# yongduosui/CAL

Measured on AMD Instinct MI355X. Metric: graphs/sec (train step) on SPMotif b=0.9 batch=128, higher is better.
Workload: dtype f32; 1 GPU; spmotif_b0.9_causalgcn_h128_l3_bs128; model=CausalGCN, batch_per_gpu=128, global_batch=128, hidden=128, layers=3, node_num=7, launch=graph(8 steps per graph launch, remainder 3), parallelism=dp1, resident_batches=8

## Files before the change

### cal_amd/csrc/engine.hip

```cpp
#include <string.h>
#include <hip/hip_ext.h>

#include <algorithm>
#include <type_traits>
#include <vector>

#include "engine_kernels.hpp"
#include "engine_readout.hpp"
#include "engine_gconv.hpp"
#include "engine_gconv_bwd.hpp"
#include "engine_ggat.hpp"
#include "engine_plan.hpp"
#include "engine_attbwd.hpp"
#include "engine_ro_step.hpp"
#include "engine_gin.hpp"
#include "engine_ggin.hpp"
#include "engine_feat.hpp"
#include "engine_gwide.hpp"
#include "engine_attwide.hpp"

namespace cal {

constexpr int MAX_LAYERS = 6;
constexpr int MAX_SLABS = 24;
// ... 129 lines not shown
    int o_cw, o_cb, o_ow, o_ob;
    int o_fc1_w[3], o_fc1_b[3], o_fc2_w[3], o_fc2_b[3];
    BNSlot bn[MAX_LAYERS + 9];
    int nbn;
    int a_convb[MAX_LAYERS], a_cb, a_ob, a_dwn, a_dwe, a_db1, a_db2, a_sync, arena_n, bn_plane;
    char* ws; size_t ws_bytes;
    int64_t capN, capE, capB;
    float *h, *z, *zco, *hco, *anode, *pq, *att, *dis_unit, *dis_co, *pooled, *pcnt, *xco, *y1, *zl, *logp, *stats, *zpart;
    int adam_fused;
    int ro_rows;
    int striped;
    int fold_zero;
    int bn0_dirty_host;
    int gwide;
    int ro_step;
    float *dzl, *dyh1, *dy1, *dxh, *dpool, *dZco, *gn, *gself, *ddeg, *dl, *dzco, *dXhco, *dZ, *dzi, *dXh, *slabs;
    size_t slab_floats;
    double* arena;
    double* parts; size_t parts_doubles;
    hipStream_t side; hipEvent_t ev_fork[24], ev_join[24];
    int *rowptr_dst, *nbr_dst, *eid_dst, *rowptr_src, *nbr_src, *eid_src, *row32, *col32, *work, *status, *gptr, *iperm, *eptr;
    float* wslot;
    float* coef_src;
    float* coef;
    int max_nodes, max_edges;
    const int64_t *node_ptr, *edge_ptr;
    const int64_t* tile_gptr; int ntiles;
    int K; float gat_p, gat_slope;
    uint64_t gat_seed[MAX_LAYERS];
    unsigned long long* gat_ctr;
// ... 26 lines not shown
              hipStream_t stream);
}

extern "C" int64_t cal_gat_bwd_ws(int64_t N, int64_t E, int64_t K, int64_t D);

CAL_EXPORT void* cal_engine_create(int64_t F, int64_t H, int64_t C, int64_t L) {
    if (H % 4 != 0 || H > 256 || H < 4 || L < 0 || L > MAX_LAYERS || F < 1 || C < 1 || C > 64) {
        set_error("cal_engine_create: unsupported shape (need hidden %% 4 == 0, hidden <= 256, layers <= %d, classes <= 64)", MAX_LAYERS);
        return nullptr;
    }
    Engine* e = new Engine();
    memset(e, 0, sizeof(Engine));
    if (hipHostMalloc((void**)&e->host_status, 64, hipHostMallocMapped | hipHostMallocCoherent) == hipSuccess) *e->host_status = 0;
    else { (void)hipGetLastError(); e->host_status = nullptr; }
    { const char* v = getenv("CAL_AMD_RO_STEP"); e->ro_step = !(v && v[0] == '0'); }
    { const char* v = getenv("CAL_AMD_RO_ROWS"); e->ro_rows = !(v && v[0] == '0'); }
    { const char* v = getenv("CAL_AMD_STRIPED"); e->striped = !(v && v[0] == '0'); }
    { const char* v = getenv("CAL_AMD_GWIDE"); e->gwide = !(v && v[0] == '0'); }
    { const char* v = getenv("CAL_AMD_FOLD_ZERO"); e->fold_zero = !(v && v[0] == '0'); }
    e->bn0_dirty_host = 1;
    {
        int dev = 0, cus = 0;
        if (hipGetDevice(&dev) != hipSuccess || hipDeviceGetAttribute(&cus, hipDeviceAttributeMultiprocessorCount, dev) != hipSuccess) cus = 0;
        if (cus < 3 * ((int)H / RO_CW) + 8) e->ro_step = 0;
        e->num_cus = cus > 0 ? cus : 256;
        if (cus < 3 * ((int)H / RO_CW) * RBK_MAXRB + 8) e->ro_rows = 0;
    }
    { const char* v = getenv("CAL_AMD_ADAM_FUSED"); e->adam_fused = !(v && v[0] == '0'); }
    e->F = (int)F; e->H = (int)H; e->C = (int)C; e->L = (int)L;
    e->loop_w = 1.f;
// ... 950 lines not shown
    SpmmBranch b0{e->zco, e->hco, e->P + e->o_cb, e->att, e->dis_co, Acc(), Acc(), nullptr, nullptr, nullptr};
    SpmmBranch b1{e->zco + NH, e->hco + NH, e->P + e->o_ob, e->att + E, e->dis_co + N, Acc(), Acc(), nullptr, nullptr, nullptr};
    RC(launch_espmm(st, gd, SpmmBranch2{{b0, b1}}, 2, 1, e->loop_w, N, H, spmm_rpb(H, false)));
    CAL_CHECK_LAUNCH("k_espmm(co)"); STAGE();
    RC(launch_pool2(c)); STAGE();
    return 0;
}

int fwd_readout(Ctx& c) {
    Engine* e = c.e;
    const int B = c.B, H = e->H, C = e->C, L = e->L;
    hipStream_t st = c.st;
    if (c.r.ro == Readout::OneLaunch || c.r.ro == Readout::Rows) {
        RoStepArgs sa;
        memset(&sa, 0, sizeof(sa));
        sa.a = make_ro(c); sa.zpart = e->zpart; sa.sync = reinterpret_cast<int*>(e->arena + e->a_sync); sa.status = e->status;
        if (c.r.ro == Readout::OneLaunch) {
            hipLaunchKernelGGL(k_ro_step<false>, dim3(3, H / RO_CW), dim3(256), 0, st, sa);
        } else {
            const int nrb = cdiv(B, RS_B), nch = H / RO_CW;
            sa.nrb = nrb;
            sa.xch = parts_alloc(c, (size_t)3 * nch * RBK_XCH);
            if (!sa.xch) return no_parts();
            sa.gw1_slab = e->slabs; sa.gw2_slab = e->slabs + (size_t)3 * nrb * H * H;
            hipLaunchKernelGGL(k_ro_step<true>, dim3(3, nch, nrb), dim3(256), 0, st, sa);
        }
        CAL_CHECK_LAUNCH("k_ro_step"); STAGE();
        return 0;
    }
    if (c.r.ro == Readout::FourKernel) {
        const RoArgs ra = make_ro(c);
        hipLaunchKernelGGL(k_ro_fwd_a, dim3(3, H / RO_CW), dim3(256), 0, st, ra);
        CAL_CHECK_LAUNCH("k_ro_fwd_a"); STAGE();
        hipLaunchKernelGGL(k_ro_fwd_b, dim3(3, cdiv(B, RO_RB)), dim3(256), 0, st, ra);
        CAL_CHECK_LAUNCH("k_ro_fwd_b"); STAGE();
        if (!c.want_grad) {
            hipLaunchKernelGGL(k_ro_loss, dim3(3), dim3(256), 0, st, ra);
            CAL_CHECK_LAUNCH("k_ro_loss");
        }
        return 0;
// ... 982 lines not shown
```

### cal_amd/csrc/engine_ro_step.hpp

```cpp
#pragma once
#include "engine_readout.hpp"

namespace cal {

constexpr int RS_B = 128;
constexpr int RS_K = 128;
constexpr int RS_LD = RS_K + 4;

struct RoStepArgs {
    RoArgs a;
    float* zpart;
    int* sync;
    int* status;
    double* xch;
    float* gw1_slab; float* gw2_slab;
    int nrb;
};
constexpr int RBK_MAXRB = 4;
constexpr int RBK_N0 = 2 * RS_K, RBK_N1 = 2 * RO_CW, RBK_N2 = 2 * (RO_CW + 1), RBK_N3 = 4 * 64;
constexpr int RBK_O1 = RBK_MAXRB * RBK_N0, RBK_O2 = RBK_O1 + RBK_MAXRB * RBK_N1, RBK_O3 = RBK_O2 + RBK_MAXRB * RBK_N2;
constexpr int RBK_XCH = RBK_O3 + RBK_MAXRB * RBK_N3;
constexpr int RBK_SYNC_INTS = 3 * RBK_MAXRB * 2 + 3 * (RS_K / RO_CW) * 4;

__device__ __forceinline__ void ro_step_arrive(int* ctr) {
// ... 3 lines not shown
__device__ __forceinline__ void ro_step_wait(int* ctr, int n, int* status) {
    if (threadIdx.x == 0) {
        int spins = 0;
        while (__hip_atomic_load(ctr, __ATOMIC_RELAXED, __HIP_MEMORY_SCOPE_AGENT) < n) {
            if (++spins > (1 << 21)) { if (status) atomicOr(status, 256); break; }
            __builtin_amdgcn_s_sleep(1);
        }
        __builtin_amdgcn_fence(__ATOMIC_ACQUIRE, "agent");
    }
    __syncthreads();
}
__device__ __forceinline__ void ro_step_barrier(int* ctr, int n, int* status) {
    ro_step_arrive(ctr);
    ro_step_wait(ctr, n, status);
}
template <int NT, bool BN>
__device__ __forceinline__ void ro_mfma_rowk_nt(int kred, const float* X, int ld, int nrow, const float* Wr, const float* sc,
                                                const float* sh, ro_f32x4 (&acc)[4]) {
    const int l = threadIdx.x & 63, w = threadIdx.x >> 6, lr = l & 15, lk = l >> 4;
    const float* ar[NT];
#pragma unroll
    for (int t = 0; t < NT; ++t) ar[t] = X + min((w + 4 * t) * 16 + lr, nrow - 1) * ld + 4 * lk;
    const float* br = Wr + lr * ld + 4 * lk;
    float4 a4[NT], b4, s4 = make_float4(1.f, 1.f, 1.f, 1.f), h4 = make_float4(0.f, 0.f, 0.f, 0.f);
    auto fetch = [&](int k0, float4 (&a)[NT], float4& b, float4& s, float4& h) {
#pragma unroll
        for (int t = 0; t < NT; ++t) a[t] = *reinterpret_cast<const float4*>(ar[t] + k0);
        b = *reinterpret_cast<const float4*>(br + k0);
        if (BN) { s = *reinterpret_cast<const float4*>(sc + k0 + 4 * lk); h = *reinterpret_cast<const float4*>(sh + k0 + 4 * lk); }
    };
    fetch(0, a4, b4, s4, h4);
    for (int k0 = 0; k0 < kred; k0 += 16) {
        float4 an[NT], bn, sn = s4, hn = h4;
        fetch(min(k0 + 16, kred - 16), an, bn, sn, hn);
        const float bb[4] = {b4.x, b4.y, b4.z, b4.w}, ss[4] = {s4.x, s4.y, s4.z, s4.w}, hh[4] = {h4.x, h4.y, h4.z, h4.w};
#pragma unroll
        for (int j = 0; j < 4; ++j)
#pragma unroll
            for (int t = 0; t < NT; ++t) {
                const float aa[4] = {a4[t].x, a4[t].y, a4[t].z, a4[t].w};
                acc[t] = __builtin_amdgcn_mfma_f32_16x16x4f32(BN ? fmaf(aa[j], ss[j], hh[j]) : aa[j], bb[j], acc[t], 0, 0, 0);
            }
#pragma unroll
        for (int t = 0; t < NT; ++t) a4[t] = an[t];
        b4 = bn; s4 = sn; h4 = hn;
    }
}
template <bool BN>
__device__ __forceinline__ void ro_mfma_rowk(int ntiles, int kred, const float* X, int ld, int nrow, const float* Wr, const float* sc,
                                             const float* sh, ro_f32x4 (&acc)[4]) {
    switch ((ntiles + 3) / 4) {
        case 1: ro_mfma_rowk_nt<1, BN>(kred, X, ld, nrow, Wr, sc, sh, acc); break;
        case 2: ro_mfma_rowk_nt<2, BN>(kred, X, ld, nrow, Wr, sc, sh, acc); break;
        case 3: ro_mfma_rowk_nt<3, BN>(kred, X, ld, nrow, Wr, sc, sh, acc); break;
        default: ro_mfma_rowk_nt<4, BN>(kred, X, ld, nrow, Wr, sc, sh, acc); break;
    }
}

template <int NV>
__device__ __forceinline__ void rbk_total(double (&v)[NV], int t, int n, double* xs, int nrb, int rb, int* ctr, int* status) {
    if (t < n) {
#pragma unroll
        for (int q = 0; q < NV; ++q) xs[(size_t)rb * NV * n + q * n + t] = v[q];
    }
    ro_step_barrier(ctr, nrb, status);
    if (t < n) {
#pragma unroll
        for (int q = 0; q < NV; ++q) {
            double tot = 0.0;
            for (int r = 0; r < nrb; ++r) tot += xs[(size_t)r * NV * n + q * n + t];
            v[q] = tot;
        }
    }
}

template <bool RBK>
__global__ void __launch_bounds__(256) k_ro_step(const RoStepArgs sa) {
    warm_kernargs<(sizeof(RoStepArgs) < 1024 ? sizeof(RoStepArgs) : 1024)>();
    const RoArgs& a = sa.a;
    __shared__ __attribute__((aligned(16))) float Xs[RS_B * RS_LD];
    __shared__ __attribute__((aligned(16))) float Ws[RO_CW * RS_LD];
    __shared__ __attribute__((aligned(16))) float W1t[RO_CW * RS_LD];
    __shared__ __attribute__((aligned(16))) float scratch[2 * RS_B * RO_CW];
    __shared__ __attribute__((aligned(16))) float xn[RS_B * RO_CW];
    __shared__ __attribute__((aligned(16))) float y1c[RS_B * RO_CW];
    __shared__ __attribute__((aligned(16))) float zs[2048];
    __shared__ __attribute__((aligned(16))) float W2c[64 * RO_CW];
    __shared__ __attribute__((aligned(16))) float sc_s[RS_K], sh_s[RS_K], mean1_s[RS_K], rstd1_s[RS_K];
    __shared__ int perm_s[256];
    __shared__ double red[2][256];
    __shared__ float c2[6][RO_CW];
    __shared__ double lossp_s[2];
    const int hd = blockIdx.x, ch = blockIdx.y, j0 = ch * RO_CW, nch = gridDim.y;
    const int Bt = a.B, rb = RBK ? (int)blockIdx.z : 0, r0 = rb * RS_B, nrb = RBK ? sa.nrb : 1;
    const int B = RBK ? min(RS_B, Bt - r0) : Bt, K = a.H, C = a.C, ld = RS_LD, K4 = K / 4, BC = B * C, BCt = Bt * C;
    int* const cbar = RBK ? sa.sync + (hd * RBK_MAXRB + rb) * 2 : sa.sync + hd * 2;
    int* const gbar = sa.sync + 3 * RBK_MAXRB * 2 + (hd * nch + ch) * 4;
    double* const xch = RBK ? sa.xch + (size_t)(hd * nch + ch) * RBK_XCH : nullptr;
    const RoHead& h = a.h[hd];
    const int l = threadIdx.x & 63, w = threadIdx.x >> 6, j = l & 15, lk = l >> 4;
    const int rl = threadIdx.x / RO_CW;
    float* dyh = scratch;
    float* yn = scratch + RS_B * RO_CW;
    double (*red8)[256] = reinterpret_cast<double (*)[256]>(scratch);
    const int B16 = (B + 15) & ~15, ntiles = B16 / 16;
    const bool duty_out = ch == 1 % nch, duty_loss = ch == 2 % nch, duty_db2 = ch == 3 % nch,
               duty_xco = ch == 4 % nch, duty_run1 = ch == 5 % nch;

    RO_CLK(40);
    const bool colfix = 256 % K4 == 0;
    float sf[4] = {0.f, 0.f, 0.f, 0.f}, qf[4] = {0.f, 0.f, 0.f, 0.f}, pvt[4] = {0.f, 0.f, 0.f, 0.f};
    int nst = 0;
    auto add_stats = [&](const float4 v) {
        const float vv[4] = {v.x, v.y, v.z, v.w};
#pragma unroll
        for (int c = 0; c < 4; ++c) {
            pvt[c] = nst == 0 ? vv[c] : pvt[c];
            const float d = vv[c] - pvt[c];
            sf[c] += d; qf[c] = fmaf(d, d, qf[c]);
        }
        ++nst;
    };
    int pv = hd == 2 ? (int)a.perm[r0 + min((int)threadIdx.x, B - 1)] : 0;
    float g2 = h.bn2.gamma[j0 + j], b2n = h.bn2.beta[j0 + j], rm2 = h.bn2.run_mean[j0 + j], rv2 = h.bn2.run_var[j0 + j];
    float bias1 = h.b1[j0 + j];
    float rm1 = h.bn1.run_mean[min((int)threadIdx.x, K - 1)], rv1 = h.bn1.run_var[min((int)threadIdx.x, K - 1)];
    int ylab = (int)a.y[r0 + min((int)threadIdx.x, B - 1)];
    {
        RoBatch<float4, 2> bw;
        RoBatch<float, 8> bt;
        RoBatch<float, 4> bw2;
        ro_issue(bw, RO_CW, K4, [&](int jj, int c) { return *reinterpret_cast<const float4*>(h.W1 + (size_t)(j0 + jj) * K + c * 4); });
        ro_issue(bt, K, RO_CW, [&](int jj, int ii) { return h.W1[(size_t)jj * K + j0 + ii]; });
        ro_issue(bw2, C, RO_CW, [&](int c, int jj) { return h.W2[(size_t)c * K + j0 + jj]; });
        auto commit_weights = [&]() {
            ro_commit(bw, RO_CW, K4, [&](int jj, int c, const float4 v) { *reinterpret_cast<float4*>(Ws + jj * ld + c * 4) = v; });
            ro_commit(bt, K, RO_CW, [&](int jj, int ii, float v) { W1t[ii * ld + jj] = v; });
            ro_commit(bw2, C, RO_CW, [&](int c, int jj, float v) { W2c[c * RO_CW + jj] = v; });
            asm volatile("" : "+v"(g2), "+v"(b2n), "+v"(rm2), "+v"(rv2), "+v"(bias1), "+v"(ylab), "+v"(rm1), "+v"(rv1));
        };
        RoBatch<float4, 16> bx;
        if (hd == 2) {
            asm volatile("" : "+v"(pv));
            perm_s[threadIdx.x] = pv;
            __syncthreads();
            RoBatch<float4, 16> bp;
            ro_issue(bx, B, K4, [&](int b, int c) { return *reinterpret_cast<const float4*>(a.pooled + (size_t)(Bt + r0 + b) * K + c * 4); });
            ro_issue(bp, B, K4, [&](int b, int c) { return *reinterpret_cast<const float4*>(a.pooled + (size_t)perm_s[b] * K + c * 4); });
            commit_weights();
            ro_commit2(bx, bp, B, K4, [&](int b, int c, const float4 o, const float4 p) {
                const float4 v = make_float4(p.x + o.x, p.y + o.y, p.z + o.z, p.w + o.w);
                *reinterpret_cast<float4*>(Xs + b * ld + c * 4) = v;
                if (colfix) add_stats(v);
                if (duty_xco) *reinterpret_cast<float4*>(a.xco + (size_t)(r0 + b) * K + c * 4) = v;
            });
            if (duty_xco && (int)threadIdx.x < B) a.iperm[pv] = r0 + threadIdx.x;
        } else {
            const float* src = a.pooled + (hd == 0 ? (size_t)0 : (size_t)Bt * K) + (size_t)r0 * K;
            ro_issue(bx, B, K4, [&](int b, int c) { return *reinterpret_cast<const float4*>(src + (size_t)b * K + c * 4); });
            commit_weights();
            ro_commit(bx, B, K4, [&](int b, int c, const float4 v) {
                *reinterpret_cast<float4*>(Xs + b * ld + c * 4) = v;
                if (colfix) add_stats(v);
            });
        }
        __syncthreads();
    }
    RO_CLK(41);
    {
        const int np = 256 / K4, cg = threadIdx.x % K4, part = threadIdx.x / K4;
        if (!colfix && part < np) {
#pragma unroll 4
            for (int b = part; b < B; b += np) add_stats(*reinterpret_cast<const float4*>(Xs + b * ld + 4 * cg));
        }
#pragma unroll
        for (int c = 0; c < 4; ++c) {
            const double P = (double)pvt[c], S0 = (double)sf[c], n0 = (double)nst;
            red8[c][threadIdx.x] = S0 + n0 * P;
            red8[4 + c][threadIdx.x] = (double)qf[c] + 2.0 * P * S0 + n0 * P * P;
        }
        __syncthreads();
        double SQ[2] = {0.0, 0.0};
        if ((int)threadIdx.x < K) {
            const int g = threadIdx.x >> 2, c = threadIdx.x & 3;
            for (int p = 0; p < np; ++p) { SQ[0] += red8[c][p * K4 + g]; SQ[1] += red8[4 + c][p * K4 + g]; }
        }
        if (RBK) rbk_total<2>(SQ, threadIdx.x, K, xch, nrb, rb, gbar + 0, sa.status);
        if ((int)threadIdx.x < K) {
            const int k = threadIdx.x;
            const double S = SQ[0], Q = SQ[1];
            float sc, sh, mean, rstd;
            ro_bn_from_sums(h.bn1, k, S, Q, sc, sh, mean, rstd);
            sc_s[k] = sc; sh_s[k] = sh; mean1_s[k] = mean; rstd1_s[k] = rstd;
            if (duty_run1 && rb == 0) {
                const double m = S * (double)h.bn1.inv_n;
                double v = Q * (double)h.bn1.inv_n - m * m;
                if (v < 0.0) v = 0.0;
                h.bn1.run_mean[k] = 0.9f * rm1 + 0.1f * (float)m;
                h.bn1.run_var[k] = 0.9f * rv1 + 0.1f * (float)(v * (double)h.bn1.unbias);
                if (k == 0 && h.bn1.nbt) *h.bn1.nbt += 1;
            }
        }
        __syncthreads();
    }
    RO_CLK(42);
    for (int idx = threadIdx.x; idx < B16 * RO_CW; idx += 256) {
        const int b = idx / RO_CW, ii = idx % RO_CW;
        xn[idx] = b < B ? Xs[b * ld + j0 + ii] : 0.f;
    }
    ro_f32x4 acc[4] = {};
    ro_mfma_rowk<true>(ntiles, K, Xs, ld, B, Ws, sc_s, sh_s, acc);
    float s1 = 0.f, s2 = 0.f, pv2 = 0.f;
    int n2 = 0;
#pragma unroll
    for (int t = 0; t < 4; ++t)
#pragma unroll
        for (int r = 0; r < 4; ++r) {
            const int b = (w + 4 * t) * 16 + lk * 4 + r;
            const float v = b < B ? fmaxf(acc[t][r] + bias1, 0.f) : 0.f;
            if (b < B) y1c[b * RO_CW + j] = v;
            pv2 = (b < B && n2 == 0) ? v : pv2;
            const float d = b < B ? v - pv2 : 0.f;
            n2 += b < B ? 1 : 0;
            s1 += d; s2 = fmaf(d, d, s2);
        }
    RO_CLK(43);
    {
        const double P = (double)pv2, S0 = (double)s1, n0 = (double)n2;
        red[0][threadIdx.x] = S0 + n0 * P; red[1][threadIdx.x] = (double)s2 + 2.0 * P * S0 + n0 * P * P;
    }
    __syncthreads();
    double SQ2[2] = {0.0, 0.0};
    if (threadIdx.x < RO_CW)
        for (int p = 0; p < 16; ++p) { SQ2[0] += red[0][p * RO_CW + threadIdx.x]; SQ2[1] += red[1][p * RO_CW + threadIdx.x]; }
    if (RBK) rbk_total<2>(SQ2, threadIdx.x, RO_CW, xch + RBK_O1, nrb, rb, gbar + 1, sa.status);
    if (threadIdx.x < RO_CW) {
        const double S = SQ2[0], Q = SQ2[1];
        if (rb == 0) { h.st2_sum[j0 + threadIdx.x] = S; h.st2_sq[j0 + threadIdx.x] = Q; }
        const double m = S * (double)h.bn2.inv_n;
        double v = Q * (double)h.bn2.inv_n - m * m;
        if (v < 0.0) v = 0.0;
        c2[0][threadIdx.x] = (float)m; c2[1][threadIdx.x] = 1.0f / sqrtf((float)v + h.bn2.eps);
        c2[2][threadIdx.x] = g2; c2[3][threadIdx.x] = b2n;
        if (rb == 0) {
            h.bn2.run_mean[j0 + threadIdx.x] = 0.9f * rm2 + 0.1f * (float)m;
            h.bn2.run_var[j0 + threadIdx.x] = 0.9f * rv2 + 0.1f * (float)(v * (double)h.bn2.unbias);
            if (ch == 0 && threadIdx.x == 0 && h.bn2.nbt) *h.bn2.nbt += 1;
        }
    }
    __syncthreads();
    const float mean2 = c2[0][j], rstd2 = c2[1][j], gam2 = c2[2][j], bet2 = c2[3][j];
    {
        const float sc = gam2 * rstd2, sh = bet2 - mean2 * sc;
        for (int b = rl; b < B; b += 16) yn[b * RO_CW + j] = fmaf(y1c[b * RO_CW + j], sc, sh);
    }
    __syncthreads();
    {
        float* zp = sa.zpart + ((size_t)hd * nch + ch) * BCt + (size_t)r0 * C;
        for (int o = threadIdx.x; o < BC; o += 256) {
            const int b = o / C, c = o % C;
            const float4* yr = reinterpret_cast<const float4*>(yn + b * RO_CW);
            const float4* wr = reinterpret_cast<const float4*>(W2c + c * RO_CW);
            zp[o] = dot4(yr[3], wr[3], dot4(yr[2], wr[2], dot4(yr[1], wr[1], dot4(yr[0], wr[0], 0.f))));
        }
    }
    RO_CLK(44);
    ro_step_barrier(cbar, nch, sa.status);
    RO_CLK(45);

    for (int o0 = 0; o0 < BC; o0 += 512) {
        float pz[2][8], bz[2];
#pragma unroll
        for (int v = 0; v < 2; ++v) {
            const int o = min(o0 + v * 256 + (int)threadIdx.x, BC - 1);
            bz[v] = h.b2[o % C];
#pragma unroll
            for (int p = 0; p < 8; ++p) pz[v][p] = sa.zpart[((size_t)hd * nch + min(p, nch - 1)) * BCt + (size_t)r0 * C + o];
        }
#pragma unroll
        for (int v = 0; v < 2; ++v) {
            ro_pin(bz[v]);
#pragma unroll
            for (int p = 0; p < 8; ++p) ro_pin(pz[v][p]);
        }
#pragma unroll
        for (int v = 0; v < 2; ++v) {
            const int o = o0 + v * 256 + (int)threadIdx.x;
            float z = 0.f;
#pragma unroll
            for (int p = 0; p < 8; ++p) z += p < nch ? pz[v][p] : 0.f;
            z += bz[v];
            if (o < BC) {
                zs[o] = z;
                if (duty_out) a.zl[(size_t)hd * BCt + (size_t)r0 * C + o] = z;
            }
        }
    }
    __syncthreads();
    float lv = 0.f, cv = 0.f;
    if ((int)threadIdx.x < B) {
        const int b = threadIdx.x;
        const float u = 1.0f / (float)C, invB = 1.0f / (float)Bt, logu = logf(u);
// ... 30 lines not shown
            for (int k = 0; k < C; ++k) m = fmaxf(m, zr[k]);
            float se = 0.f;
            for (int k = 0; k < C; ++k) se += expf(zr[k] - m);
            const float lse = m + logf(se);
            for (int k = 0; k < C; ++k) finish(k, zr[k], lse);
        }
        lv = (float)lrow; cv = arg == yy ? 1.f : 0.f;
    }
    if (duty_loss) {
        double ls = (double)lv, cs = (double)cv;
#pragma unroll
        for (int o = 32; o > 0; o >>= 1) { ls += __shfl_xor(ls, o, 64); cs += __shfl_xor(cs, o, 64); }
        if (l == 0) { red[0][w] = ls; red[1][w] = cs; }
        __syncthreads();
        if (threadIdx.x == 0) {
            const double lsum = red[0][0] + red[0][1] + red[0][2] + red[0][3], csum = red[1][0] + red[1][1] + red[1][2] + red[1][3];
            if (RBK) { lossp_s[0] = lsum; lossp_s[1] = csum; }
            else {
                a.stats[1 + hd] = (float)(lsum / (double)Bt);
                a.stats[hd == 1 ? 4 : (hd == 0 ? 5 : 6)] = (float)csum;
            }
        }
    }
    __syncthreads();
    RO_CLK(46);
    const float* dzs = zs;
    double db1_keep = 0.0, db2_keep = 0.0;
    {
        float t1f = 0.f, t2f = 0.f;
        float dq[8] = {0.f, 0.f, 0.f, 0.f, 0.f, 0.f, 0.f, 0.f};
        for (int c = 0; c < C; ++c) {
            const float wc2 = W2c[c * RO_CW + j];
            float dzv[8];
#pragma unroll
            for (int qq = 0; qq < 8; ++qq) dzv[qq] = dzs[min(rl + 16 * qq, B - 1) * C + c];
#pragma unroll
            for (int qq = 0; qq < 8; ++qq) dq[qq] = fmaf(dzv[qq], wc2, dq[qq]);
        }
#pragma unroll
        for (int qq = 0; qq < 8; ++qq) {
            const int b = rl + 16 * qq;
            const float yv = y1c[min(b, B - 1) * RO_CW + j];
            if (b < B) {
                const float n = (yv - mean2) * rstd2;
                dyh[b * RO_CW + j] = dq[qq];
                t1f += dq[qq]; t2f = fmaf(dq[qq], n, t2f);
            }
        }
        double t1 = (double)t1f, t2 = (double)t2f;
        red[0][threadIdx.x] = t1; red[1][threadIdx.x] = t2;
        __syncthreads();
        if (rl == 0) for (int p = 1; p < 16; ++p) { t1 += red[0][p * RO_CW + j]; t2 += red[1][p * RO_CW + j]; }
        if (RBK) {
            double tt[2] = {rl == 0 ? t1 : 0.0, rl == 0 ? t2 : 0.0};
            if (threadIdx.x == RO_CW) { tt[0] = duty_loss ? lossp_s[0] : 0.0; tt[1] = duty_loss ? lossp_s[1] : 0.0; }
            rbk_total<2>(tt, threadIdx.x, RO_CW + 1, xch + RBK_O2, nrb, rb, gbar + 2, sa.status);
            t1 = tt[0]; t2 = tt[1];
            if (threadIdx.x == RO_CW && duty_loss && rb == 0) {
                a.stats[1 + hd] = (float)(tt[0] / (double)Bt);
                a.stats[hd == 1 ? 4 : (hd == 0 ? 5 : 6)] = (float)tt[1];
            }
        }
        if (rl == 0) {
            if (rb == 0) { h.d2_sum[j0 + j] = t1; h.d2_prod[j0 + j] = t2; }
            c2[4][j] = (float)(t1 * (double)h.bn2.inv_n); c2[5][j] = (float)(t2 * (double)h.bn2.inv_n);
        }
        __syncthreads();
        const float m1 = c2[4][j], m2 = c2[5][j], gs = gam2 * rstd2;
        float sbf = 0.f;
#pragma unroll
        for (int qq = 0; qq < 8; ++qq) {
            const int b = rl + 16 * qq;
            if (b < B) {
                const float yv = y1c[b * RO_CW + j];
                const float n = (yv - mean2) * rstd2;
                const float dy = yv > 0.f ? gs * (dyh[b * RO_CW + j] - m1 - n * m2) : 0.f;
                a.dy1[((size_t)hd * Bt + r0 + b) * K + j0 + j] = dy;
                sbf += dy;
            }
        }
        double sb = (double)sbf;
        red[0][threadIdx.x] = sb;
        __syncthreads();
        if (rl == 0) {
            for (int p = 1; p < 16; ++p) sb += red[0][p * RO_CW + j];
            if (RBK) db1_keep = sb; else h.db1[j0 + j] = sb;
        }
    }
    RO_CLK(47);
    ro_step_arrive(cbar + 1);
    RO_CLK(48);
    ro_step_wait(cbar + 1, nch, sa.status);
    RO_CLK(49);
    float* Ds = Xs;
    RoBatch<float4, 16> bd;
    ro_issue(bd, B, K4, [&](int b, int c) { return *reinterpret_cast<const float4*>(a.dy1 + ((size_t)hd * Bt + r0 + b) * K + c * 4); });
    if (duty_db2) {
        const int np = 256 / C, c = threadIdx.x % C, part = threadIdx.x / C;
        double sdz = 0.0;
        if (part < np) for (int b = part; b < B; b += np) sdz += (double)dzs[b * C + c];
        red[0][threadIdx.x] = sdz;
        __syncthreads();
        if (part == 0) {
            for (int p2 = 1; p2 < np; ++p2) sdz += red[0][p2 * C + c];
            if (RBK) db2_keep = sdz; else h.db2[c] = sdz;
        }
        __syncthreads();
    }
    {
        const int nout = C * RO_CW;
        float* fred = dyh;
        for (int o0 = 0; o0 < nout; o0 += 256) {
            const int no = min(256, nout - o0), np = 256 / no;
            const int o = o0 + threadIdx.x % no, part = threadIdx.x / no;
            const int c = o / RO_CW, jj = o % RO_CW;
            float accw = 0.f;
            if (part < np) {
#pragma unroll 4
                for (int b = part; b < B; b += np) accw = fmaf(dzs[b * C + c], yn[b * RO_CW + jj], accw);
            }
            __syncthreads();
            fred[threadIdx.x] = accw;
            __syncthreads();
            if (part == 0) {
                for (int p = 1; p < np; ++p) accw += fred[p * no + threadIdx.x];
                (RBK ? sa.gw2_slab + ((size_t)hd * nrb + rb) * C * K : h.gW2)[(size_t)c * K + j0 + jj] = accw;
            }
        }
    }
    ro_commit(bd, B, K4, [&](int b, int c, const float4 v) { *reinterpret_cast<float4*>(Ds + b * ld + c * 4) = v; });
    for (int idx = threadIdx.x; idx < (B16 - B) * ld; idx += 256) Ds[B * ld + idx] = 0.f;
    __syncthreads();
    RO_CLK(50);
    const int i = j, i0 = j0;
    const float mean1 = mean1_s[i0 + i], rstd1 = rstd1_s[i0 + i], gs1 = sc_s[i0 + i], sh1 = sh_s[i0 + i];
    ro_f32x4 dacc[4] = {};
    ro_mfma_rowk<false>(ntiles, K, Ds, ld, B, W1t, nullptr, nullptr, dacc);
    float u1 = 0.f, u2 = 0.f;
#pragma unroll
    for (int t = 0; t < 4; ++t)
#pragma unroll
        for (int r = 0; r < 4; ++r) {
            const int b = (w + 4 * t) * 16 + lk * 4 + r;
            const float n = (xn[min(b, B16 - 1) * RO_CW + i] - mean1) * rstd1;
            const float dv = b < B ? dacc[t][r] : 0.f;
            u1 += dv; u2 = fmaf(dv, n, u2);
        }
    red[0][threadIdx.x] = (double)u1; red[1][threadIdx.x] = (double)u2;
    __syncthreads();
    {
        double uu[4] = {0.0, 0.0, 0.0, 0.0};
        if (threadIdx.x < RO_CW)
            for (int p = 0; p < 16; ++p) { uu[0] += red[0][p * RO_CW + threadIdx.x]; uu[1] += red[1][p * RO_CW + threadIdx.x]; }
        if (RBK) {
            uu[2] = threadIdx.x < RO_CW ? db1_keep : 0.0;
            uu[3] = (duty_db2 && (int)threadIdx.x < C) ? db2_keep : 0.0;
            rbk_total<4>(uu, threadIdx.x, 64, xch + RBK_O3, nrb, rb, gbar + 3, sa.status);
            if (rb == 0) {
                if (threadIdx.x < RO_CW) h.db1[j0 + threadIdx.x] = uu[2];
                if (duty_db2 && (int)threadIdx.x < C) h.db2[threadIdx.x] = uu[3];
            }
        }
        if (threadIdx.x < RO_CW) {
            const double S = uu[0], Q = uu[1];
            if (rb == 0) { h.d1_sum[i0 + threadIdx.x] = S; h.d1_prod[i0 + threadIdx.x] = Q; }
            c2[4][threadIdx.x] = (float)(S * (double)h.bn1.inv_n); c2[5][threadIdx.x] = (float)(Q * (double)h.bn1.inv_n);
        }
    }
    __syncthreads();
    {
        const float m1 = c2[4][i], m2 = c2[5][i];
#pragma unroll
        for (int t = 0; t < 4; ++t)
#pragma unroll
            for (int r = 0; r < 4; ++r) {
                const int b = (w + 4 * t) * 16 + lk * 4 + r;
                if (b < B) {
                    const float xr = xn[b * RO_CW + i];
                    const float n = (xr - mean1) * rstd1;
                    a.dxin[((size_t)hd * Bt + r0 + b) * K + i0 + i] = gs1 * (dacc[t][r] - m1 - n * m2);
                    xn[b * RO_CW + i] = fmaf(xr, gs1, sh1);
                }
            }
    }
    __syncthreads();
    RO_CLK(51);
    ro_f32x4 wacc[4] = {};
    ro_mfma_tiles(K / 16, B16, [&](int row, int k) { return Ds[k * ld + min(row, K - 1)]; },
                  [&](int k, int col) { return xn[k * RO_CW + col]; }, wacc);
#pragma unroll
    for (int t = 0; t < 4; ++t)
        if (w + 4 * t < K / 16) {
#pragma unroll
            for (int r = 0; r < 4; ++r)
                (RBK ? sa.gw1_slab + ((size_t)hd * nrb + rb) * K * K : h.gW1)[(size_t)((w + 4 * t) * 16 + lk * 4 + r) * K + i0 + i] = wacc[t][r];
        }
    RO_CLK(52);
}

}
```

Before: 580,400 graphs/s.

## Run readout step kernel with 8 waves, splitting MFMA K-reduction across wave halves

Templates k_ro_step on block size and adds a 512-thread variant, selected by default for the single-launch readout when batch exceeds 64. The two wave groups each compute half of the K (or batch) reduction in the MFMA GEMMs and combine partial accumulators through shared memory. Loads and reductions are re-strided to NT threads. This aims to cut the latency of a low-occupancy kernel that runs only 3×(H/RO_CW) blocks, at the cost of extra shared-memory combine passes and barriers.

```diff
diff --git a/cal_amd/csrc/engine.hip b/cal_amd/csrc/engine.hip
--- a/cal_amd/csrc/engine.hip
+++ b/cal_amd/csrc/engine.hip
@@ -167,6 +167,7 @@
     int bn0_dirty_host;
     int gwide;
     int ro_step;
+    int ro_step_nt;
     float *dzl, *dyh1, *dy1, *dxh, *dpool, *dZco, *gn, *gself, *ddeg, *dl, *dzco, *dXhco, *dZ, *dzi, *dXh, *slabs;
     size_t slab_floats;
     double* arena;
@@ -223,6 +224,7 @@
     if (hipHostMalloc((void**)&e->host_status, 64, hipHostMallocMapped | hipHostMallocCoherent) == hipSuccess) *e->host_status = 0;
     else { (void)hipGetLastError(); e->host_status = nullptr; }
     { const char* v = getenv("CAL_AMD_RO_STEP"); e->ro_step = !(v && v[0] == '0'); }
+    { const char* v = getenv("CAL_AMD_RO_STEP_NT"); const int n = v ? atoi(v) : 0; e->ro_step_nt = n == 256 || n == 512 ? n : 0; }
     { const char* v = getenv("CAL_AMD_RO_ROWS"); e->ro_rows = !(v && v[0] == '0'); }
     { const char* v = getenv("CAL_AMD_STRIPED"); e->striped = !(v && v[0] == '0'); }
     { const char* v = getenv("CAL_AMD_GWIDE"); e->gwide = !(v && v[0] == '0'); }
@@ -1203,16 +1205,19 @@
     if (c.r.ro == Readout::OneLaunch || c.r.ro == Readout::Rows) {
         RoStepArgs sa;
         memset(&sa, 0, sizeof(sa));
+        const int nt = e->ro_step_nt ? e->ro_step_nt : (c.r.ro == Readout::OneLaunch && B > RS_B / 2 ? 512 : 256);
         sa.a = make_ro(c); sa.zpart = e->zpart; sa.sync = reinterpret_cast<int*>(e->arena + e->a_sync); sa.status = e->status;
         if (c.r.ro == Readout::OneLaunch) {
-            hipLaunchKernelGGL(k_ro_step<false>, dim3(3, H / RO_CW), dim3(256), 0, st, sa);
+            if (nt == 512) hipLaunchKernelGGL((k_ro_step<false, 512>), dim3(3, H / RO_CW), dim3(512), 0, st, sa);
+            else hipLaunchKernelGGL((k_ro_step<false, 256>), dim3(3, H / RO_CW), dim3(256), 0, st, sa);
         } else {
             const int nrb = cdiv(B, RS_B), nch = H / RO_CW;
             sa.nrb = nrb;
             sa.xch = parts_alloc(c, (size_t)3 * nch * RBK_XCH);
             if (!sa.xch) return no_parts();
             sa.gw1_slab = e->slabs; sa.gw2_slab = e->slabs + (size_t)3 * nrb * H * H;
-            hipLaunchKernelGGL(k_ro_step<true>, dim3(3, nch, nrb), dim3(256), 0, st, sa);
+            if (nt == 512) hipLaunchKernelGGL((k_ro_step<true, 512>), dim3(3, nch, nrb), dim3(512), 0, st, sa);
+            else hipLaunchKernelGGL((k_ro_step<true, 256>), dim3(3, nch, nrb), dim3(256), 0, st, sa);
         }
         CAL_CHECK_LAUNCH("k_ro_step"); STAGE();
         return 0;
diff --git a/cal_amd/csrc/engine_ro_step.hpp b/cal_amd/csrc/engine_ro_step.hpp
--- a/cal_amd/csrc/engine_ro_step.hpp
+++ b/cal_amd/csrc/engine_ro_step.hpp
@@ -41,46 +41,60 @@
     ro_step_arrive(ctr);
     ro_step_wait(ctr, n, status);
 }
-template <int NT, bool BN>
-__device__ __forceinline__ void ro_mfma_rowk_nt(int kred, const float* X, int ld, int nrow, const float* Wr, const float* sc,
-                                                const float* sh, ro_f32x4 (&acc)[4]) {
-    const int l = threadIdx.x & 63, w = threadIdx.x >> 6, lr = l & 15, lk = l >> 4;
-    const float* ar[NT];
-#pragma unroll
-    for (int t = 0; t < NT; ++t) ar[t] = X + min((w + 4 * t) * 16 + lr, nrow - 1) * ld + 4 * lk;
-    const float* br = Wr + lr * ld + 4 * lk;
-    float4 a4[NT], b4, s4 = make_float4(1.f, 1.f, 1.f, 1.f), h4 = make_float4(0.f, 0.f, 0.f, 0.f);
-    auto fetch = [&](int k0, float4 (&a)[NT], float4& b, float4& s, float4& h) {
-#pragma unroll
-        for (int t = 0; t < NT; ++t) a[t] = *reinterpret_cast<const float4*>(ar[t] + k0);
+template <int TW, bool BN>
+__device__ __forceinline__ void ro_mfma_rowk_nt(int wq, int kbeg, int kred, const float* X, int ld, int nrow, const float* Wr,
+                                                const float* sc, const float* sh, ro_f32x4 (&acc)[4]) {
+    const int l = threadIdx.x & 63, lr = l & 15, lk = l >> 4;
+    const float* ar[TW];
+#pragma unroll
+    for (int t = 0; t < TW; ++t) ar[t] = X + min((wq + 4 * t) * 16 + lr, nrow - 1) * ld + kbeg + 4 * lk;
+    const float* br = Wr + lr * ld + kbeg + 4 * lk;
+    if (BN) { sc += kbeg + 4 * lk; sh += kbeg + 4 * lk; }
+    float4 a4[TW], b4, s4 = make_float4(1.f, 1.f, 1.f, 1.f), h4 = make_float4(0.f, 0.f, 0.f, 0.f);
+    auto fetch = [&](int k0, float4 (&a)[TW], float4& b, float4& s, float4& h) {
+#pragma unroll
+        for (int t = 0; t < TW; ++t) a[t] = *reinterpret_cast<const float4*>(ar[t] + k0);
         b = *reinterpret_cast<const float4*>(br + k0);
-        if (BN) { s = *reinterpret_cast<const float4*>(sc + k0 + 4 * lk); h = *reinterpret_cast<const float4*>(sh + k0 + 4 * lk); }
+        if (BN) { s = *reinterpret_cast<const float4*>(sc + k0); h = *reinterpret_cast<const float4*>(sh + k0); }
     };
     fetch(0, a4, b4, s4, h4);
     for (int k0 = 0; k0 < kred; k0 += 16) {
-        float4 an[NT], bn, sn = s4, hn = h4;
+        float4 an[TW], bn, sn = s4, hn = h4;
         fetch(min(k0 + 16, kred - 16), an, bn, sn, hn);
         const float bb[4] = {b4.x, b4.y, b4.z, b4.w}, ss[4] = {s4.x, s4.y, s4.z, s4.w}, hh[4] = {h4.x, h4.y, h4.z, h4.w};
 #pragma unroll
         for (int j = 0; j < 4; ++j)
 #pragma unroll
-            for (int t = 0; t < NT; ++t) {
+            for (int t = 0; t < TW; ++t) {
                 const float aa[4] = {a4[t].x, a4[t].y, a4[t].z, a4[t].w};
                 acc[t] = __builtin_amdgcn_mfma_f32_16x16x4f32(BN ? fmaf(aa[j], ss[j], hh[j]) : aa[j], bb[j], acc[t], 0, 0, 0);
             }
 #pragma unroll
-        for (int t = 0; t < NT; ++t) a4[t] = an[t];
+        for (int t = 0; t < TW; ++t) a4[t] = an[t];
         b4 = bn; s4 = sn; h4 = hn;
     }
 }
 template <bool BN>
-__device__ __forceinline__ void ro_mfma_rowk(int ntiles, int kred, const float* X, int ld, int nrow, const float* Wr, const float* sc,
-                                             const float* sh, ro_f32x4 (&acc)[4]) {
+__device__ __forceinline__ void ro_mfma_rowk(int wq, int ntiles, int kbeg, int kred, const float* X, int ld, int nrow, const float* Wr,
+                                             const float* sc, const float* sh, ro_f32x4 (&acc)[4]) {
     switch ((ntiles + 3) / 4) {
-        case 1: ro_mfma_rowk_nt<1, BN>(kred, X, ld, nrow, Wr, sc, sh, acc); break;
-        case 2: ro_mfma_rowk_nt<2, BN>(kred, X, ld, nrow, Wr, sc, sh, acc); break;
-        case 3: ro_mfma_rowk_nt<3, BN>(kred, X, ld, nrow, Wr, sc, sh, acc); break;
-        default: ro_mfma_rowk_nt<4, BN>(kred, X, ld, nrow, Wr, sc, sh, acc); break;
+        case 1: ro_mfma_rowk_nt<1, BN>(wq, kbeg, kred, X, ld, nrow, Wr, sc, sh, acc); break;
+        case 2: ro_mfma_rowk_nt<2, BN>(wq, kbeg, kred, X, ld, nrow, Wr, sc, sh, acc); break;
+        case 3: ro_mfma_rowk_nt<3, BN>(wq, kbeg, kred, X, ld, nrow, Wr, sc, sh, acc); break;
+        default: ro_mfma_rowk_nt<4, BN>(wq, kbeg, kred, X, ld, nrow, Wr, sc, sh, acc); break;
+    }
+}
+
+__device__ __forceinline__ void ro_half_combine(int wq, int kh, int ntw, float* park, ro_f32x4 (&acc)[4]) {
+    ro_f32x4* slot = reinterpret_cast<ro_f32x4*>(park) + (wq * 4) * 64 + (threadIdx.x & 63);
+    if (kh == 1) {
+#pragma unroll
+        for (int t = 0; t < 4; ++t) if (t < ntw) slot[t * 64] = acc[t];
+    }
+    __syncthreads();
+    if (kh == 0) {
+#pragma unroll
+        for (int t = 0; t < 4; ++t) if (t < ntw) acc[t] += slot[t * 64];
     }
 }
 
@@ -101,8 +115,11 @@
     }
 }
 
-template <bool RBK>
-__global__ void __launch_bounds__(256) k_ro_step(const RoStepArgs sa) {
+template <bool RBK, int NT>
+__global__ void __launch_bounds__(NT) k_ro_step(const RoStepArgs sa) {
+    static_assert(NT == 256 || NT == 512, "k_ro_step: 4 or 8 waves");
+    constexpr int NRP = NT / RO_CW;
+    constexpr int XU = RS_B * (RS_K / 4) / NT;
     warm_kernargs<(sizeof(RoStepArgs) < 1024 ? sizeof(RoStepArgs) : 1024)>();
     const RoArgs& a = sa.a;
     __shared__ __attribute__((aligned(16))) float Xs[RS_B * RS_LD];
@@ -114,8 +131,8 @@
     __shared__ __attribute__((aligned(16))) float zs[2048];
     __shared__ __attribute__((aligned(16))) float W2c[64 * RO_CW];
     __shared__ __attribute__((aligned(16))) float sc_s[RS_K], sh_s[RS_K], mean1_s[RS_K], rstd1_s[RS_K];
-    __shared__ int perm_s[256];
-    __shared__ double red[2][256];
+    __shared__ int perm_s[RS_B];
+    __shared__ double red[2][NT];
     __shared__ float c2[6][RO_CW];
     __shared__ double lossp_s[2];
     const int hd = blockIdx.x, ch = blockIdx.y, j0 = ch * RO_CW, nch = gridDim.y;
@@ -126,16 +143,19 @@
     double* const xch = RBK ? sa.xch + (size_t)(hd * nch + ch) * RBK_XCH : nullptr;
     const RoHead& h = a.h[hd];
     const int l = threadIdx.x & 63, w = threadIdx.x >> 6, j = l & 15, lk = l >> 4;
+    const int wq = w & 3, kh = NT == 512 ? w >> 2 : 0;
+    const bool own = kh == 0;
     const int rl = threadIdx.x / RO_CW;
     float* dyh = scratch;
     float* yn = scratch + RS_B * RO_CW;
-    double (*red8)[256] = reinterpret_cast<double (*)[256]>(scratch);
-    const int B16 = (B + 15) & ~15, ntiles = B16 / 16;
+    double (*red8s)[NT] = reinterpret_cast<double (*)[NT]>(scratch);
+    auto red8q = [&](int c) { return reinterpret_cast<double*>(c < 2 ? xn : y1c) + (c & 1) * NT; };
+    const int B16 = (B + 15) & ~15, ntiles = B16 / 16, ntw = (ntiles + 3) / 4;
     const bool duty_out = ch == 1 % nch, duty_loss = ch == 2 % nch, duty_db2 = ch == 3 % nch,
                duty_xco = ch == 4 % nch, duty_run1 = ch == 5 % nch;
 
     RO_CLK(40);
-    const bool colfix = 256 % K4 == 0;
+    const bool colfix = NT % K4 == 0;
     float sf[4] = {0.f, 0.f, 0.f, 0.f}, qf[4] = {0.f, 0.f, 0.f, 0.f}, pvt[4] = {0.f, 0.f, 0.f, 0.f};
     int nst = 0;
     auto add_stats = [&](const float4 v) {
@@ -154,28 +174,28 @@
     float rm1 = h.bn1.run_mean[min((int)threadIdx.x, K - 1)], rv1 = h.bn1.run_var[min((int)threadIdx.x, K - 1)];
     int ylab = (int)a.y[r0 + min((int)threadIdx.x, B - 1)];
     {
-        RoBatch<float4, 2> bw;
-        RoBatch<float, 8> bt;
-        RoBatch<float, 4> bw2;
-        ro_issue(bw, RO_CW, K4, [&](int jj, int c) { return *reinterpret_cast<const float4*>(h.W1 + (size_t)(j0 + jj) * K + c * 4); });
-        ro_issue(bt, K, RO_CW, [&](int jj, int ii) { return h.W1[(size_t)jj * K + j0 + ii]; });
-        ro_issue(bw2, C, RO_CW, [&](int c, int jj) { return h.W2[(size_t)c * K + j0 + jj]; });
+        RoBatch<float4, 512 / NT> bw;
+        RoBatch<float, 2048 / NT> bt;
+        RoBatch<float, 1024 / NT> bw2;
+        ro_issue<NT>(bw, RO_CW, K4, [&](int jj, int c) { return *reinterpret_cast<const float4*>(h.W1 + (size_t)(j0 + jj) * K + c * 4); });
+        ro_issue<NT>(bt, K, RO_CW, [&](int jj, int ii) { return h.W1[(size_t)jj * K + j0 + ii]; });
+        ro_issue<NT>(bw2, C, RO_CW, [&](int c, int jj) { return h.W2[(size_t)c * K + j0 + jj]; });
         auto commit_weights = [&]() {
-            ro_commit(bw, RO_CW, K4, [&](int jj, int c, const float4 v) { *reinterpret_cast<float4*>(Ws + jj * ld + c * 4) = v; });
-            ro_commit(bt, K, RO_CW, [&](int jj, int ii, float v) { W1t[ii * ld + jj] = v; });
-            ro_commit(bw2, C, RO_CW, [&](int c, int jj, float v) { W2c[c * RO_CW + jj] = v; });
+            ro_commit<NT>(bw, RO_CW, K4, [&](int jj, int c, const float4 v) { *reinterpret_cast<float4*>(Ws + jj * ld + c * 4) = v; });
+            ro_commit<NT>(bt, K, RO_CW, [&](int jj, int ii, float v) { W1t[ii * ld + jj] = v; });
+            ro_commit<NT>(bw2, C, RO_CW, [&](int c, int jj, float v) { W2c[c * RO_CW + jj] = v; });
             asm volatile("" : "+v"(g2), "+v"(b2n), "+v"(rm2), "+v"(rv2), "+v"(bias1), "+v"(ylab), "+v"(rm1), "+v"(rv1));
         };
-        RoBatch<float4, 16> bx;
+        RoBatch<float4, XU> bx;
         if (hd == 2) {
             asm volatile("" : "+v"(pv));
-            perm_s[threadIdx.x] = pv;
+            if (threadIdx.x < RS_B) perm_s[threadIdx.x] = pv;
             __syncthreads();
-            RoBatch<float4, 16> bp;
-            ro_issue(bx, B, K4, [&](int b, int c) { return *reinterpret_cast<const float4*>(a.pooled + (size_t)(Bt + r0 + b) * K + c * 4); });
-            ro_issue(bp, B, K4, [&](int b, int c) { return *reinterpret_cast<const float4*>(a.pooled + (size_t)perm_s[b] * K + c * 4); });
+            RoBatch<float4, XU> bp;
+            ro_issue<NT>(bx, B, K4, [&](int b, int c) { return *reinterpret_cast<const float4*>(a.pooled + (size_t)(Bt + r0 + b) * K + c * 4); });
+            ro_issue<NT>(bp, B, K4, [&](int b, int c) { return *reinterpret_cast<const float4*>(a.pooled + (size_t)perm_s[b] * K + c * 4); });
             commit_weights();
-            ro_commit2(bx, bp, B, K4, [&](int b, int c, const float4 o, const float4 p) {
+            ro_commit2<NT>(bx, bp, B, K4, [&](int b, int c, const float4 o, const float4 p) {
                 const float4 v = make_float4(p.x + o.x, p.y + o.y, p.z + o.z, p.w + o.w);
                 *reinterpret_cast<float4*>(Xs + b * ld + c * 4) = v;
                 if (colfix) add_stats(v);
@@ -184,9 +204,9 @@
             if (duty_xco && (int)threadIdx.x < B) a.iperm[pv] = r0 + threadIdx.x;
         } else {
             const float* src = a.pooled + (hd == 0 ? (size_t)0 : (size_t)Bt * K) + (size_t)r0 * K;
-            ro_issue(bx, B, K4, [&](int b, int c) { return *reinterpret_cast<const float4*>(src + (size_t)b * K + c * 4); });
+            ro_issue<NT>(bx, B, K4, [&](int b, int c) { return *reinterpret_cast<const float4*>(src + (size_t)b * K + c * 4); });
             commit_weights();
-            ro_commit(bx, B, K4, [&](int b, int c, const float4 v) {
+            ro_commit<NT>(bx, B, K4, [&](int b, int c, const float4 v) {
                 *reinterpret_cast<float4*>(Xs + b * ld + c * 4) = v;
                 if (colfix) add_stats(v);
             });
@@ -195,7 +215,7 @@
     }
     RO_CLK(41);
     {
-        const int np = 256 / K4, cg = threadIdx.x % K4, part = threadIdx.x / K4;
+        const int np = NT / K4, cg = threadIdx.x % K4, part = threadIdx.x / K4;
         if (!colfix && part < np) {
 #pragma unroll 4
             for (int b = part; b < B; b += np) add_stats(*reinterpret_cast<const float4*>(Xs + b * ld + 4 * cg));
@@ -203,14 +223,15 @@
 #pragma unroll
         for (int c = 0; c < 4; ++c) {
             const double P = (double)pvt[c], S0 = (double)sf[c], n0 = (double)nst;
-            red8[c][threadIdx.x] = S0 + n0 * P;
-            red8[4 + c][threadIdx.x] = (double)qf[c] + 2.0 * P * S0 + n0 * P * P;
+            red8s[c][threadIdx.x] = S0 + n0 * P;
+            red8q(c)[threadIdx.x] = (double)qf[c] + 2.0 * P * S0 + n0 * P * P;
         }
         __syncthreads();
         double SQ[2] = {0.0, 0.0};
         if ((int)threadIdx.x < K) {
             const int g = threadIdx.x >> 2, c = threadIdx.x & 3;
-            for (int p = 0; p < np; ++p) { SQ[0] += red8[c][p * K4 + g]; SQ[1] += red8[4 + c][p * K4 + g]; }
+            const double* rq = red8q(c);
+            for (int p = 0; p < np; ++p) { SQ[0] += red8s[c][p * K4 + g]; SQ[1] += rq[p * K4 + g]; }
         }
         if (RBK) rbk_total<2>(SQ, threadIdx.x, K, xch, nrb, rb, gbar + 0, sa.status);
         if ((int)threadIdx.x < K) {
@@ -231,28 +252,31 @@
         __syncthreads();
     }
     RO_CLK(42);
-    for (int idx = threadIdx.x; idx < B16 * RO_CW; idx += 256) {
+    for (int idx = threadIdx.x; idx < B16 * RO_CW; idx += NT) {
         const int b = idx / RO_CW, ii = idx % RO_CW;
         xn[idx] = b < B ? Xs[b * ld + j0 + ii] : 0.f;
     }
     ro_f32x4 acc[4] = {};
-    ro_mfma_rowk<true>(ntiles, K, Xs, ld, B, Ws, sc_s, sh_s, acc);
+    const int klo = NT == 512 ? ((K / 16 + 1) >> 1) * 16 : K, kbeg = kh * klo, klen = kh ? K - klo : klo;
+    if (klen > 0) ro_mfma_rowk<true>(wq, ntiles, kbeg, klen, Xs, ld, B, Ws, sc_s, sh_s, acc);
+    if (NT == 512) ro_half_combine(wq, kh, ntw, scratch, acc);
     float s1 = 0.f, s2 = 0.f, pv2 = 0.f;
     int n2 = 0;
 #pragma unroll
     for (int t = 0; t < 4; ++t)
 #pragma unroll
         for (int r = 0; r < 4; ++r) {
-            const int b = (w + 4 * t) * 16 + lk * 4 + r;
-            const float v = b < B ? fmaxf(acc[t][r] + bias1, 0.f) : 0.f;
-            if (b < B) y1c[b * RO_CW + j] = v;
-            pv2 = (b < B && n2 == 0) ? v : pv2;
-            const float d = b < B ? v - pv2 : 0.f;
-            n2 += b < B ? 1 : 0;
+            const int b = (wq + 4 * t) * 16 + lk * 4 + r;
+            const bool in = own && b < B;
+            const float v = in ? fmaxf(acc[t][r] + bias1, 0.f) : 0.f;
+            if (in) y1c[b * RO_CW + j] = v;
+            pv2 = (in && n2 == 0) ? v : pv2;
+            const float d = in ? v - pv2 : 0.f;
+            n2 += in ? 1 : 0;
             s1 += d; s2 = fmaf(d, d, s2);
         }
     RO_CLK(43);
-    {
+    if (own) {
         const double P = (double)pv2, S0 = (double)s1, n0 = (double)n2;
         red[0][threadIdx.x] = S0 + n0 * P; red[1][threadIdx.x] = (double)s2 + 2.0 * P * S0 + n0 * P * P;
     }
@@ -279,12 +303,12 @@
     const float mean2 = c2[0][j], rstd2 = c2[1][j], gam2 = c2[2][j], bet2 = c2[3][j];
     {
         const float sc = gam2 * rstd2, sh = bet2 - mean2 * sc;
-        for (int b = rl; b < B; b += 16) yn[b * RO_CW + j] = fmaf(y1c[b * RO_CW + j], sc, sh);
+        for (int b = rl; b < B; b += NRP) yn[b * RO_CW + j] = fmaf(y1c[b * RO_CW + j], sc, sh);
     }
     __syncthreads();
     {
         float* zp = sa.zpart + ((size_t)hd * nch + ch) * BCt + (size_t)r0 * C;
-        for (int o = threadIdx.x; o < BC; o += 256) {
+        for (int o = threadIdx.x; o < BC; o += NT) {
             const int b = o / C, c = o % C;
             const float4* yr = reinterpret_cast<const float4*>(yn + b * RO_CW);
             const float4* wr = reinterpret_cast<const float4*>(W2c + c * RO_CW);
@@ -295,24 +319,25 @@
     ro_step_barrier(cbar, nch, sa.status);
     RO_CLK(45);
 
+    constexpr int ZV = 512 / NT;
     for (int o0 = 0; o0 < BC; o0 += 512) {
-        float pz[2][8], bz[2];
-#pragma unroll
-        for (int v = 0; v < 2; ++v) {
-            const int o = min(o0 + v * 256 + (int)threadIdx.x, BC - 1);
+        float pz[ZV][8], bz[ZV];
+#pragma unroll
+        for (int v = 0; v < ZV; ++v) {
+            const int o = min(o0 + v * NT + (int)threadIdx.x, BC - 1);
             bz[v] = h.b2[o % C];
 #pragma unroll
             for (int p = 0; p < 8; ++p) pz[v][p] = sa.zpart[((size_t)hd * nch + min(p, nch - 1)) * BCt + (size_t)r0 * C + o];
         }
 #pragma unroll
-        for (int v = 0; v < 2; ++v) {
+        for (int v = 0; v < ZV; ++v) {
             ro_pin(bz[v]);
 #pragma unroll
             for (int p = 0; p < 8; ++p) ro_pin(pz[v][p]);
         }
 #pragma unroll
-        for (int v = 0; v < 2; ++v) {
-            const int o = o0 + v * 256 + (int)threadIdx.x;
+        for (int v = 0; v < ZV; ++v) {
+            const int o = o0 + v * NT + (int)threadIdx.x;
             float z = 0.f;
 #pragma unroll
             for (int p = 0; p < 8; ++p) z += p < nch ? pz[v][p] : 0.f;
@@ -373,7 +398,9 @@
         if (l == 0) { red[0][w] = ls; red[1][w] = cs; }
         __syncthreads();
         if (threadIdx.x == 0) {
-            const double lsum = red[0][0] + red[0][1] + red[0][2] + red[0][3], csum = red[1][0] + red[1][1] + red[1][2] + red[1][3];
+            double lsum = 0.0, csum = 0.0;
+#pragma unroll
+            for (int q = 0; q < NT / 64; ++q) { lsum += red[0][q]; csum += red[1][q]; }
             if (RBK) { lossp_s[0] = lsum; lossp_s[1] = csum; }
             else {
                 a.stats[1 + hd] = (float)(lsum / (double)Bt);
@@ -386,19 +413,20 @@
     const float* dzs = zs;
     double db1_keep = 0.0, db2_keep = 0.0;
     {
+        constexpr int RPL = RS_B / NRP;
         float t1f = 0.f, t2f = 0.f;
-        float dq[8] = {0.f, 0.f, 0.f, 0.f, 0.f, 0.f, 0.f, 0.f};
+        float dq[RPL] = {};
         for (int c = 0; c < C; ++c) {
             const float wc2 = W2c[c * RO_CW + j];
-            float dzv[8];
-#pragma unroll
-            for (int qq = 0; qq < 8; ++qq) dzv[qq] = dzs[min(rl + 16 * qq, B - 1) * C + c];
-#pragma unroll
-            for (int qq = 0; qq < 8; ++qq) dq[qq] = fmaf(dzv[qq], wc2, dq[qq]);
-        }
-#pragma unroll
-        for (int qq = 0; qq < 8; ++qq) {
-            const int b = rl + 16 * qq;
+            float dzv[RPL];
+#pragma unroll
+            for (int qq = 0; qq < RPL; ++qq) dzv[qq] = dzs[min(rl + NRP * qq, B - 1) * C + c];
+#pragma unroll
+            for (int qq = 0; qq < RPL; ++qq) dq[qq] = fmaf(dzv[qq], wc2, dq[qq]);
+        }
+#pragma unroll
+        for (int qq = 0; qq < RPL; ++qq) {
+            const int b = rl + NRP * qq;
             const float yv = y1c[min(b, B - 1) * RO_CW + j];
             if (b < B) {
                 const float n = (yv - mean2) * rstd2;
@@ -409,7 +437,7 @@
         double t1 = (double)t1f, t2 = (double)t2f;
         red[0][threadIdx.x] = t1; red[1][threadIdx.x] = t2;
         __syncthreads();
-        if (rl == 0) for (int p = 1; p < 16; ++p) { t1 += red[0][p * RO_CW + j]; t2 += red[1][p * RO_CW + j]; }
+        if (rl == 0) for (int p = 1; p < NRP; ++p) { t1 += red[0][p * RO_CW + j]; t2 += red[1][p * RO_CW + j]; }
         if (RBK) {
             double tt[2] = {rl == 0 ? t1 : 0.0, rl == 0 ? t2 : 0.0};
             if (threadIdx.x == RO_CW) { tt[0] = duty_loss ? lossp_s[0] : 0.0; tt[1] = duty_loss ? lossp_s[1] : 0.0; }
@@ -428,8 +456,8 @@
         const float m1 = c2[4][j], m2 = c2[5][j], gs = gam2 * rstd2;
         float sbf = 0.f;
 #pragma unroll
-        for (int qq = 0; qq < 8; ++qq) {
-            const int b = rl + 16 * qq;
+        for (int qq = 0; qq < RPL; ++qq) {
+            const int b = rl + NRP * qq;
             if (b < B) {
                 const float yv = y1c[b * RO_CW + j];
                 const float n = (yv - mean2) * rstd2;
@@ -442,7 +470,7 @@
         red[0][threadIdx.x] = sb;
         __syncthreads();
         if (rl == 0) {
-            for (int p = 1; p < 16; ++p) sb += red[0][p * RO_CW + j];
+            for (int p = 1; p < NRP; ++p) sb += red[0][p * RO_CW + j];
             if (RBK) db1_keep = sb; else h.db1[j0 + j] = sb;
         }
     }
@@ -452,10 +480,10 @@
     ro_step_wait(cbar + 1, nch, sa.status);
     RO_CLK(49);
     float* Ds = Xs;
-    RoBatch<float4, 16> bd;
-    ro_issue(bd, B, K4, [&](int b, int c) { return *reinterpret_cast<const float4*>(a.dy1 + ((size_t)hd * Bt + r0 + b) * K + c * 4); });
+    RoBatch<float4, XU> bd;
+    ro_issue<NT>(bd, B, K4, [&](int b, int c) { return *reinterpret_cast<const float4*>(a.dy1 + ((size_t)hd * Bt + r0 + b) * K + c * 4); });
     if (duty_db2) {
-        const int np = 256 / C, c = threadIdx.x % C, part = threadIdx.x / C;
+        const int np = NT / C, c = threadIdx.x % C, part = threadIdx.x / C;
         double sdz = 0.0;
         if (part < np) for (int b = part; b < B; b += np) sdz += (double)dzs[b * C + c];
         red[0][threadIdx.x] = sdz;
@@ -469,8 +497,8 @@
     {
         const int nout = C * RO_CW;
         float* fred = dyh;
-        for (int o0 = 0; o0 < nout; o0 += 256) {
-            const int no = min(256, nout - o0), np = 256 / no;
+        for (int o0 = 0; o0 < nout; o0 += NT) {
+            const int no = min(NT, nout - o0), np = NT / no;
             const int o = o0 + threadIdx.x % no, part = threadIdx.x / no;
             const int c = o / RO_CW, jj = o % RO_CW;
             float accw = 0.f;
@@ -487,25 +515,26 @@
             }
         }
     }
-    ro_commit(bd, B, K4, [&](int b, int c, const float4 v) { *reinterpret_cast<float4*>(Ds + b * ld + c * 4) = v; });
-    for (int idx = threadIdx.x; idx < (B16 - B) * ld; idx += 256) Ds[B * ld + idx] = 0.f;
+    ro_commit<NT>(bd, B, K4, [&](int b, int c, const float4 v) { *reinterpret_cast<float4*>(Ds + b * ld + c * 4) = v; });
+    for (int idx = threadIdx.x; idx < (B16 - B) * ld; idx += NT) Ds[B * ld + idx] = 0.f;
     __syncthreads();
     RO_CLK(50);
     const int i = j, i0 = j0;
     const float mean1 = mean1_s[i0 + i], rstd1 = rstd1_s[i0 + i], gs1 = sc_s[i0 + i], sh1 = sh_s[i0 + i];
     ro_f32x4 dacc[4] = {};
-    ro_mfma_rowk<false>(ntiles, K, Ds, ld, B, W1t, nullptr, nullptr, dacc);
+    if (klen > 0) ro_mfma_rowk<false>(wq, ntiles, kbeg, klen, Ds, ld, B, W1t, nullptr, nullptr, dacc);
+    if (NT == 512) ro_half_combine(wq, kh, ntw, scratch, dacc);
     float u1 = 0.f, u2 = 0.f;
 #pragma unroll
     for (int t = 0; t < 4; ++t)
 #pragma unroll
         for (int r = 0; r < 4; ++r) {
-            const int b = (w + 4 * t) * 16 + lk * 4 + r;
+            const int b = (wq + 4 * t) * 16 + lk * 4 + r;
             const float n = (xn[min(b, B16 - 1) * RO_CW + i] - mean1) * rstd1;
-            const float dv = b < B ? dacc[t][r] : 0.f;
+            const float dv = own && b < B ? dacc[t][r] : 0.f;
             u1 += dv; u2 = fmaf(dv, n, u2);
         }
-    red[0][threadIdx.x] = (double)u1; red[1][threadIdx.x] = (double)u2;
+    if (own) { red[0][threadIdx.x] = (double)u1; red[1][threadIdx.x] = (double)u2; }
     __syncthreads();
     {
         double uu[4] = {0.0, 0.0, 0.0, 0.0};
@@ -533,8 +562,8 @@
         for (int t = 0; t < 4; ++t)
 #pragma unroll
             for (int r = 0; r < 4; ++r) {
-                const int b = (w + 4 * t) * 16 + lk * 4 + r;
-                if (b < B) {
+                const int b = (wq + 4 * t) * 16 + lk * 4 + r;
+                if (own && b < B) {
                     const float xr = xn[b * RO_CW + i];
                     const float n = (xr - mean1) * rstd1;
                     a.dxin[((size_t)hd * Bt + r0 + b) * K + i0 + i] = gs1 * (dacc[t][r] - m1 - n * m2);
@@ -545,14 +574,17 @@
     __syncthreads();
     RO_CLK(51);
     ro_f32x4 wacc[4] = {};
-    ro_mfma_tiles(K / 16, B16, [&](int row, int k) { return Ds[k * ld + min(row, K - 1)]; },
-                  [&](int k, int col) { return xn[k * RO_CW + col]; }, wacc);
+    const int blo = NT == 512 ? ((ntiles + 1) >> 1) * 16 : B16, bbeg = kh * blo, blen = kh ? B16 - blo : blo, rofs = kh * 64;
+    if (blen > 0)
+        ro_mfma_tiles(K / 16, blen, [&](int row, int k) { return Ds[(bbeg + k) * ld + min(row - rofs, K - 1)]; },
+                      [&](int k, int col) { return xn[(bbeg + k) * RO_CW + col]; }, wacc);
+    if (NT == 512) ro_half_combine(wq, kh, (K / 16 + 3) / 4, scratch, wacc);
 #pragma unroll
     for (int t = 0; t < 4; ++t)
-        if (w + 4 * t < K / 16) {
+        if (own && wq + 4 * t < K / 16) {
 #pragma unroll
             for (int r = 0; r < 4; ++r)
-                (RBK ? sa.gw1_slab + ((size_t)hd * nrb + rb) * K * K : h.gW1)[(size_t)((w + 4 * t) * 16 + lk * 4 + r) * K + i0 + i] = wacc[t][r];
+                (RBK ? sa.gw1_slab + ((size_t)hd * nrb + rb) * K * K : h.gW1)[(size_t)((wq + 4 * t) * 16 + lk * 4 + r) * K + i0 + i] = wacc[t][r];
         }
     RO_CLK(52);
 }
```

After: 583,200 graphs/s, median of 6. About the same (+0.5%).
